# sks-codes/fuzzyheavyhitters

Hardware: AMD Instinct MI355X
Metric: client×prefix key evals/sec (AES blocks/s) + full-crawl wall time, 1M clients (higher is better)
Workload: dtype u32

## Files before the change

fuzzyheavyhitters_amd/csrc/fhh_gc.hip:

```cpp
#include "fhh_internal.h"
#include "aes_keyed.h"
#include "cot_fe.h"
#include "bitslice.h"
#include "gt_window.h"

namespace fhh {

__constant__ WordTable c_T0_gc = T0;
using GcTab = Tab4T32<DevOpsX>;
constexpr int kGcThreads = 1024;

__device__ __forceinline__ void gc_fill(uint32_t* tbl) {
    for (int i = threadIdx.x; i < GcTab::kWords; i += blockDim.x) tbl[i] = GcTab::word(c_T0_gc.v, i);
    __syncthreads();
}

__device__ __forceinline__ void zero_rk(uint32_t (&rk)[11][4]) {
#pragma unroll
    for (int r = 0; r < 11; r++)
#pragma unroll
        for (int c = 0; c < 4; c++) rk[r][c] = ZERO_RK.w[r][c];
}

template <int NB>
// ... 450 lines not shown
                    } else if (t < n_act) {
                        a.gt_msgs[(uint64_t)(r - 1) * n + t] = hl ^ (o ? p1[u] : p0[u]);
                    }
                }
            }
        }
    }
}

template <int B>
__global__ __launch_bounds__(kGcThreads) void k_gt_eval(GcArgs a) {
    __shared__ uint32_t tbl_gc[GcTab::kWords];
    if ((uint64_t)blockIdx.x * kGcThreads >= gc_active(a)) return;
    gc_fill(tbl_gc);
    uint32_t b0, b1;
    GcTab::bases(threadIdx.x & 63, b0, b1);
    const uint64_t n = a.G * a.N;
    const uint64_t Npad = (uint64_t)a.nw * 64;
    const uint64_t n_act = gc_active(a);
    constexpr int U = FHH_GT_EVAL_U;
    const uint64_t stride = (uint64_t)gridDim.x * kGcThreads;
    for (uint64_t t0 = (uint64_t)blockIdx.x * kGcThreads + threadIdx.x; t0 < n_act; t0 += U * stride) {
        uint32_t h[U][4], row[U];
        uint64_t tt[U];
#pragma unroll
        for (int u = 0; u < U; u++) {
            const uint64_t t = t0 + u * stride;
            tt[u] = t;
            const uint64_t tc = t < n_act ? t : t0;
            const uint64_t g = tc / a.N;
            const uint32_t i = (uint32_t)(tc - g * a.N);
            const uint64_t tw = a.gate_base + a.g_off * a.N + tc;
            uint32_t S[4] = {0u, 0u, 0u, 0u}, r = 0;
#pragma unroll
            for (int k = B - 1; k >= 0; k--) {
                uint32_t z[4];
                ld_blk(a.ev_labels, g * B + k, Npad, i, z);
                gf_dbl(S);
#pragma unroll
                for (int c = 0; c < 4; c++) S[c] ^= z[c];
                r |= (z[0] & 1u) << k;
            }
            S[0] ^= (uint32_t)tw;
            S[1] ^= (uint32_t)(tw >> 32);
#pragma unroll
            for (int c = 0; c < 4; c++) h[u][c] = S[c];
            row[u] = r;
        }
        aes0_mmo_tab<DevOpsX, GcTab, U>(h, tbl_gc, b0, b1);
#pragma unroll
        for (int u = 0; u < U; u++) {
            const uint64_t t = tt[u];
            if (t >= n_act) continue;
            const uint64_t hl = (uint64_t)h[u][0] | ((uint64_t)h[u][1] << 32);
            a.sh_ev[t] = row[u] ? (hl ^ a.gt_msgs[(uint64_t)(row[u] - 1) * n + t])
                                : ot_fe_of_u128(hl, (uint64_t)h[u][2] | ((uint64_t)h[u][3] << 32));
        }
    }
}

template <int B>
__global__ __launch_bounds__(kGcThreads) void k_gt_garble_r32(GcArgs a) {
    __shared__ uint32_t tbl_gc[GcTab::kWords];
    if ((uint64_t)blockIdx.x * kGcThreads >= gc_active(a)) return;
    gc_fill(tbl_gc);
    uint32_t b0, b1;
    GcTab::bases(threadIdx.x & 63, b0, b1);
    constexpr uint32_t R = 1u << B;
    constexpr int NB = R < 4 ? (int)R : 4;
    const uint64_t n = a.G * a.N;
    const uint64_t Npad = (uint64_t)a.nw * 64;
    uint32_t* msgs = reinterpret_cast<uint32_t*>(a.gt_msgs);
    uint32_t* vals = reinterpret_cast<uint32_t*>(a.sh_gb);
    uint32_t Dk[B][4];
#pragma unroll
    for (int c = 0; c < 4; c++) Dk[0][c] = a.delta[c];
#pragma unroll
    for (int k = 1; k < B; k++) {
#pragma unroll
        for (int c = 0; c < 4; c++) Dk[k][c] = Dk[k - 1][c];
        gf_dbl(Dk[k]);
    }
    const uint64_t n_act = gc_active(a);
    const uint64_t stride = (uint64_t)gridDim.x * kGcThreads;
    for (uint64_t t = (uint64_t)blockIdx.x * kGcThreads + threadIdx.x; t < n_act; t += stride) {
        const uint64_t g = t / a.N;
        const uint32_t i = (uint32_t)(t - g * a.N);
        const uint64_t tw = a.gate_base + a.g_off * a.N + t;
        uint32_t S[4] = {0u, 0u, 0u, 0u}, col = 0;
#pragma unroll
        for (int k = B - 1; k >= 0; k--) {
            uint32_t z[4];
            ld_blk(a.ev_labels, g * B + k, Npad, i, z);
            const uint32_t xb = plane_bit(a.gb_planes, a.g_off + g, B, k, a.nw, i);
            gf_dbl(S);
#pragma unroll
            for (int c = 0; c < 4; c++) {
                z[c] ^= xb ? 0u : a.delta[c];
                S[c] ^= z[c];
            }
            col |= (z[0] & 1u) << k;
        }
        S[0] ^= (uint32_t)tw;
        S[1] ^= (uint32_t)(tw >> 32);
        const uint32_t rstar = ~col & (R - 1);
        uint32_t p0 = 0, p1 = 0;
#pragma unroll
        for (uint32_t pass = 0; pass < R / NB; pass++) {
            uint32_t h[NB][4];
#pragma unroll
            for (int j = 0; j < NB; j++) {
                const uint32_t flip = (pass * NB + j) ^ col;
#pragma unroll
                for (int c = 0; c < 4; c++) {
                    uint32_t w = S[c];
#pragma unroll
                    for (int k = 0; k < B; k++) w ^= ((flip >> k) & 1u) ? Dk[k][c] : 0u;
                    h[j][c] = w;
                }
            }
            aes0_mmo_tab<DevOpsX, GcTab, NB>(h, tbl_gc, b0, b1);
#pragma unroll
            for (int j = 0; j < NB; j++) {
                const uint32_t r = pass * NB + j;
                const uint32_t o = (uint32_t)(r == rstar) ^ a.mask;
                if (r == 0) {
                    const uint32_t h32 = h[0][0];
                    const uint32_t v = o == 0 ? h32 : (a.mask ? h32 - 1u : h32 + 1u);
                    p0 = v;
                    p1 = a.mask ? v + 1u : v - 1u;
                    vals[t] = a.mask ? v + 1u : v;
                } else {
                    msgs[(uint64_t)(r - 1) * n + t] = h[j][0] ^ (o ? p1 : p0);
                }
            }
        }
    }
}

template <int B>
__global__ __launch_bounds__(kGcThreads) void k_gt_eval_r32(GcArgs a) {
    __shared__ uint32_t tbl_gc[GcTab::kWords];
    if ((uint64_t)blockIdx.x * kGcThreads >= gc_active(a)) return;
    gc_fill(tbl_gc);
    uint32_t b0, b1;
    GcTab::bases(threadIdx.x & 63, b0, b1);
    const uint64_t n = a.G * a.N;
    const uint64_t Npad = (uint64_t)a.nw * 64;
    const uint64_t n_act = gc_active(a);
    const uint32_t* msgs = reinterpret_cast<const uint32_t*>(a.gt_msgs);
    uint32_t* vals = reinterpret_cast<uint32_t*>(a.sh_ev);
    constexpr int U = FHH_GT_EVAL_U;
    const uint64_t stride = (uint64_t)gridDim.x * kGcThreads;
    for (uint64_t t0 = (uint64_t)blockIdx.x * kGcThreads + threadIdx.x; t0 < n_act; t0 += U * stride) {
        uint32_t h[U][4], row[U];
        uint64_t tt[U];
#pragma unroll
        for (int u = 0; u < U; u++) {
            const uint64_t t = t0 + u * stride;
            tt[u] = t;
            const uint64_t tc = t < n_act ? t : t0;
            const uint64_t g = tc / a.N;
            const uint32_t i = (uint32_t)(tc - g * a.N);
            const uint64_t tw = a.gate_base + a.g_off * a.N + tc;
            uint32_t S[4] = {0u, 0u, 0u, 0u}, r = 0;
#pragma unroll
            for (int k = B - 1; k >= 0; k--) {
                uint32_t z[4];
                ld_blk(a.ev_labels, g * B + k, Npad, i, z);
                gf_dbl(S);
#pragma unroll
                for (int c = 0; c < 4; c++) S[c] ^= z[c];
                r |= (z[0] & 1u) << k;
            }
            S[0] ^= (uint32_t)tw;
            S[1] ^= (uint32_t)(tw >> 32);
#pragma unroll
            for (int c = 0; c < 4; c++) h[u][c] = S[c];
            row[u] = r;
        }
        aes0_mmo_tab<DevOpsX, GcTab, U>(h, tbl_gc, b0, b1);
#pragma unroll
        for (int u = 0; u < U; u++) {
            const uint64_t t = tt[u];
            if (t >= n_act) continue;
            vals[t] = row[u] ? (h[u][0] ^ msgs[(uint64_t)(row[u] - 1) * n + t]) : h[u][0];
        }
    }
}

constexpr int kRingSumThreads = 256;
constexpr uint32_t kRingSumSlice = 4096;
__global__ __launch_bounds__(kRingSumThreads) void k_ring32_child_sums(const uint32_t* vals, uint64_t n, uint64_t* sums) {
    const uint64_t c = blockIdx.y;
    const uint64_t lo = (uint64_t)blockIdx.x * kRingSumSlice;
    const uint64_t hi = lo + kRingSumSlice < n ? lo + kRingSumSlice : n;
    const uint32_t* row = vals + c * n;
    uint64_t acc = 0;
    for (uint64_t i = lo + threadIdx.x; i < hi; i += kRingSumThreads) acc += row[i];
#pragma unroll
    for (int off = 32; off > 0; off >>= 1) acc += __shfl_xor(acc, off, 64);
    if ((threadIdx.x & 63) == 0 && acc) atomicAdd(reinterpret_cast<unsigned long long*>(sums + c), (unsigned long long)acc);
}

hipError_t launch_ring32_child_sums(const uint32_t* vals, uint64_t n, uint64_t C, uint64_t* sums, hipStream_t stream) {
    if (n == 0 || C == 0) return hipSuccess;
    if (!vals || !sums) return hipErrorInvalidValue;
    const uint64_t per = (n + kRingSumSlice - 1) / kRingSumSlice;
    for (uint64_t c0 = 0; c0 < C; c0 += 65535) {
        const uint64_t cc = C - c0 < 65535 ? C - c0 : 65535;
        hipLaunchKernelGGL(k_ring32_child_sums, dim3((uint32_t)per, (uint32_t)cc), dim3(kRingSumThreads), 0, stream,
                           vals + c0 * n, n, sums + c0);
        const hipError_t e = hipGetLastError();
        if (e != hipSuccess) return e;
    }
    return hipSuccess;
}

__global__ __launch_bounds__(kRingSumThreads) void k_ring32_child_partials(const uint32_t* vals, uint64_t n, uint64_t c0,
                                                                           const LoopCtl* ctl, uint64_t g_off,
                                                                           uint64_t* partials, uint32_t slot) {
    const uint64_t c = c0 + blockIdx.y;
    if (ctl && (ctl->abort || g_off + c >= ctl->C)) return;
    const uint64_t lo = (uint64_t)blockIdx.x * kRingSumSlice;
    const uint64_t hi = lo + kRingSumSlice < n ? lo + kRingSumSlice : n;
    const uint32_t* row = vals + c * n;
    uint64_t acc = 0;
    for (uint64_t i = lo + threadIdx.x; i < hi; i += kRingSumThreads) acc += row[i];
#pragma unroll
    for (int off = 32; off > 0; off >>= 1) acc += __shfl_xor(acc, off, 64);
    if ((threadIdx.x & 63) == 0 && acc)
        atomicAdd(reinterpret_cast<unsigned long long*>(partials + (g_off + c) * 4 + slot), (unsigned long long)acc);
}

hipError_t launch_ring32_child_partials(const uint32_t* vals, uint64_t n, uint64_t G, const LoopCtl* ctl, uint64_t g_off,
                                        uint64_t* partials, uint32_t slot, hipStream_t stream) {
    if (n == 0 || G == 0) return hipSuccess;
    if (!vals || !partials) return hipErrorInvalidValue;
    const uint64_t per = (n + kRingSumSlice - 1) / kRingSumSlice;
    for (uint64_t c0 = 0; c0 < G; c0 += 65535) {
        const uint64_t cc = G - c0 < 65535 ? G - c0 : 65535;
        hipLaunchKernelGGL(k_ring32_child_partials, dim3((uint32_t)per, (uint32_t)cc), dim3(kRingSumThreads), 0, stream,
                           vals, n, c0, ctl, g_off, partials, slot);
        const hipError_t e = hipGetLastError();
        if (e != hipSuccess) return e;
    }
    return hipSuccess;
}

constexpr int kGtWaves = kGcThreads / 64;

__device__ __forceinline__ void gt_tile_round(uint32_t* st, uint32_t (&x)[32], uint32_t lane, uint32_t (&o)[2][4]) {
#pragma unroll
    for (int kk = 0; kk < 8; kk++) st[64 * kk + (lane ^ (8 * kk))] = x[kk];
    __builtin_amdgcn_wave_barrier();
    const uint32_t kk = lane & 7;
#pragma unroll
    for (int u = 0; u < 2; u++) {
        const uint32_t qq = (lane >> 3) + 8 * u;
        const uint4 v = *reinterpret_cast<const uint4*>(st + 64 * kk + ((4 * qq) ^ (8 * kk)));
        o[u][0] = v.x;
        o[u][1] = v.y;
        o[u][2] = v.z;
        o[u][3] = v.w;
    }
    __builtin_amdgcn_wave_barrier();
#pragma unroll
    for (int i = 0; i < 24; i++) x[i] = x[i + 8];
}

__device__ __forceinline__ void gt_add_partials(uint64_t* partials, uint64_t child, int k0, uint64_t lo, uint64_t hi,
                                                uint32_t lane) {
#pragma unroll
    for (int off = 32; off > 0; off >>= 1) {
        lo += __shfl_xor(lo, off, 64);
        hi += __shfl_xor(hi, off, 64);
    }
    if (lane == 0) {
        atomicAdd(reinterpret_cast<unsigned long long*>(partials + child * 4 + k0), (unsigned long long)lo);
        atomicAdd(reinterpret_cast<unsigned long long*>(partials + child * 4 + k0 + 1), (unsigned long long)hi);
    }
}

__device__ __forceinline__ uint32_t gt_tile_test(uint32_t lane, int r, int u) {
    return 256 * u + 32 * (lane >> 3) + 8 * r + (lane & 7);
}

template <int B>
__device__ __forceinline__ void gt_tile_rows(const GcArgs& a, uint64_t g, uint32_t iw, uint32_t Npt, uint32_t lane,
                                             uint32_t (&x)[32]) {
    static_assert(B >= 1 && B <= kGtTmMaxBits, "gt_tile_rows: b <= 4");
    const uint32_t q = lane >> 2, rg = lane & 3;
    if constexpr (B > kGtTmPadBits) {
        const uint32_t nw2 = 2 * a.nw;
        gt_window_fold<B>(reinterpret_cast<const uint32_t*>(a.ev_labels), g, nw2, gt_window_word(16 * iw + q, nw2), rg, x);
        transpose32(x);
        return;
    }
    const uint32_t* t0 = reinterpret_cast<const uint32_t*>(a.ev_labels) + (((uint64_t)g * B) * Npt + iw) * kGtTileWords + q;
#pragma unroll
    for (int i = 0; i < 32; i++) x[i] = __builtin_nontemporal_load(t0 + (32 * rg + i) * 16);
    if constexpr (B == 2) {
        const uint32_t* t1 = t0 + (uint64_t)Npt * kGtTileWords;
        const uint32_t y0 = __builtin_nontemporal_load(t1 + (rg ? 32 * rg - 1 : 127) * 16);
        x[0] ^= y0;
#pragma unroll
        for (int i = 1; i < 32; i++) x[i] ^= __builtin_nontemporal_load(t1 + (32 * rg + i - 1) * 16);
        if (rg == 0) {
            x[1] ^= y0;
            x[2] ^= y0;
            x[7] ^= y0;
        }
    }
    transpose32(x);
}

template <int B>
__device__ __forceinline__ void gt_tile_colours(const GcArgs& a, uint64_t g, uint32_t iw, uint32_t Npt, uint32_t lane,
                                                uint32_t (&cw)[B][2]) {
    const uint32_t* lab = reinterpret_cast<const uint32_t*>(a.ev_labels);
    if constexpr (B > kGtTmPadBits) {
#pragma unroll
        for (int k = 0; k < B; k++)
#pragma unroll
            for (int u = 0; u < 2; u++) {
                const uint32_t w = gt_window_word(16 * iw + (lane >> 3) + 8 * u, 2 * a.nw);
                cw[k][u] = lab[gt_col_offset(gt_window_col(g, B, k, 2 * a.nw, w))];
            }
        return;
    }
#pragma unroll
    for (int k = 0; k < B; k++)
#pragma unroll
        for (int u = 0; u < 2; u++)
            cw[k][u] = lab[(((uint64_t)g * B + k) * Npt + iw) * kGtTileWords + (lane >> 3) + 8 * u];
}

template <int B>
__device__ __forceinline__ uint32_t gt_row_of(const uint32_t (&cw)[B][2], int r, int u, uint32_t lane) {
    const uint32_t sh = 8 * r + (lane & 7);
    uint32_t row = 0;
#pragma unroll
    for (int k = 0; k < B; k++) row |= ((cw[k][u] >> sh) & 1u) << k;
    return row;
}

template <int B, bool GARBLER>
__device__ __forceinline__ void gt_tile_keys(const GcArgs& a, uint64_t g, uint32_t iw, uint32_t Npt, uint32_t* st,
                                             uint32_t lane, const uint32_t (&Dk)[B][4], uint32_t (&S)[8][4],
                                             uint32_t& col, uint32_t& xcol) {
    if constexpr (B > kGtTmPadBits) {
        xcol = 0;
        col = 0;
        {
            uint32_t ln = lane;
            asm volatile("" : "+v"(ln));
            uint32_t cw[B][2], nx[B][2];
            gt_tile_colours<B>(a, g, iw, Npt, ln, cw);
            if constexpr (GARBLER) {
#pragma unroll
                for (int k = 0; k < B; k++)
#pragma unroll
                    for (int u = 0; u < 2; u++) {
                        const uint32_t w = gt_window_word(16 * iw + (ln >> 3) + 8 * u, 2 * a.nw);
                        nx[k][u] = ~reinterpret_cast<const uint32_t*>(
                            a.gb_planes)[((a.g_off + g) * B + k) * (2 * (uint64_t)a.nw) + w];
                        cw[k][u] ^= nx[k][u];
                    }
            }
#pragma unroll
            for (int r = 0; r < 4; r++)
#pragma unroll
                for (int u = 0; u < 2; u++) {
                    col |= gt_row_of<B>(cw, r, u, ln) << (4 * (2 * r + u));
                    if constexpr (GARBLER) xcol |= gt_row_of<B>(nx, r, u, ln) << (4 * (2 * r + u));
                }
        }
        asm volatile("" : "+v"(col), "+v"(xcol));
        uint32_t x[32];
        gt_tile_rows<B>(a, g, iw, Npt, lane, x);
#pragma unroll 1
        for (int r = 0; r < 4; r++) {
            uint32_t o[2][4];
            gt_tile_round(st, x, lane, o);
#pragma unroll
            for (int j = 0; j < 6; j++)
#pragma unroll
                for (int c = 0; c < 4; c++) S[j][c] = S[j + 2][c];
#pragma unroll
            for (int c = 0; c < 4; c++) {
                S[6][c] = o[0][c];
                S[7][c] = o[1][c];
            }
        }
        return;
    }
    uint32_t x[32], cw[B][2], nx[B][2];
    gt_tile_rows<B>(a, g, iw, Npt, lane, x);
    gt_tile_colours<B>(a, g, iw, Npt, lane, cw);
    if constexpr (GARBLER) {
#pragma unroll
        for (int k = 0; k < B; k++)
#pragma unroll
            for (int u = 0; u < 2; u++) {
                nx[k][u] = ~reinterpret_cast<const uint32_t*>(a.gb_planes)[((a.g_off + g) * B + k) * (2 * (uint64_t)a.nw) +
                                                                          16 * iw + (lane >> 3) + 8 * u];
                cw[k][u] ^= nx[k][u];
            }
    }
    col = 0;
#pragma unroll
    for (int r = 0; r < 4; r++)
#pragma unroll
        for (int u = 0; u < 2; u++) col |= gt_row_of<B>(cw, r, u, lane) << (4 * (2 * r + u));
#pragma unroll 1
    for (int r = 0; r < 4; r++) {
        uint32_t o[2][4];
        gt_tile_round(st, x, lane, o);
        if constexpr (GARBLER) {
#pragma unroll
            for (int u = 0; u < 2; u++)
#pragma unroll
                for (int k = 0; k < B; k++) {
                    const uint32_t f = (nx[k][u] >> (8 * r + (lane & 7))) & 1u;
#pragma unroll
                    for (int c = 0; c < 4; c++) o[u][c] ^= f ? Dk[k][c] : 0u;
                }
        }
#pragma unroll
        for (int j = 0; j < 6; j++)
#pragma unroll
            for (int c = 0; c < 4; c++) S[j][c] = S[j + 2][c];
#pragma unroll
        for (int c = 0; c < 4; c++) {
            S[6][c] = o[0][c];
            S[7][c] = o[1][c];
        }
    }
}

template <int B, bool RING = false>
__global__ __launch_bounds__(kGcThreads) void k_gt_garble_tm(GcArgs a) {
    static_assert(B <= kGtTmMaxBits, "the tile-major garbler takes b <= 4");
    __shared__ uint32_t tbl_gc[GcTab::kWords];
    __shared__ __attribute__((aligned(16))) uint32_t stage[kGtWaves][512];
    const uint32_t lane = threadIdx.x & 63,
                   wv = B > kGtTmPadBits ? (uint32_t)__builtin_amdgcn_readfirstlane((int)(threadIdx.x >> 6)) : threadIdx.x >> 6;
    const uint64_t n_act = gc_active(a);
    const uint32_t Npt = (B > kGtTmPadBits ? a.nw + 7 : a.nw) / 8;
    const uint64_t tiles = (n_act / a.N) * Npt;
    if ((uint64_t)blockIdx.x * kGtWaves >= tiles) return;
    gc_fill(tbl_gc);
    uint32_t b0, b1;
    GcTab::bases(lane, b0, b1);
    constexpr uint32_t R = 1u << B;
    const uint64_t n = a.G * a.N;
    uint32_t Dk[B][4];
#pragma unroll
    for (int c = 0; c < 4; c++) Dk[0][c] = a.delta[c];
#pragma unroll
    for (int k = 1; k < B; k++) {
#pragma unroll
        for (int c = 0; c < 4; c++) Dk[k][c] = Dk[k - 1][c];
        gf_dbl(Dk[k]);
    }
    uint64_t g_next = 0, g_step = 0;
    uint32_t iw_next = 0, iw_step = 0;
    if constexpr (B > kGtTmPadBits) {
        const uint64_t w0 = (uint64_t)blockIdx.x * kGtWaves + wv, ws = (uint64_t)gridDim.x * kGtWaves;
        g_next = w0 / Npt;
        iw_next = (uint32_t)(w0 - g_next * Npt);
        g_step = ws / Npt;
        iw_step = (uint32_t)(ws - g_step * Npt);
    }
    for (uint64_t wt = (uint64_t)blockIdx.x * kGtWaves + wv; wt < tiles; wt += (uint64_t)gridDim.x * kGtWaves) {
        uint64_t g;
        uint32_t iw;
        if constexpr (B > kGtTmPadBits) {
            g = g_next;
            iw = iw_next;
            g_next += g_step;
            iw_next += iw_step;
            if (iw_next >= Npt) {
                iw_next -= Npt;
                g_next++;
            }
        } else {
            g = wt / Npt;
            iw = (uint32_t)(wt - g * Npt);
        }
        uint32_t S[8][4], col, xcol;
        gt_tile_keys<B, true>(a, g, iw, Npt, stage[wv], lane, Dk, S, col, xcol);
        uint64_t acc_lo = 0, acc_hi = 0;
        if constexpr (B > kGtTmPadBits) {
constexpr uint32_t NBW = FHH_GT_TM_WIDE_NB;
#pragma unroll 1
            for (int j = 0; j < 8; j++) {
                const uint32_t i = 512 * iw + gt_tile_test(lane, j >> 1, j & 1);
                const bool live = i < a.N;
                const uint64_t t = g * a.N + i;
                {
                    const uint64_t tw = a.gate_base + a.g_off * a.N + t;
                    S[0][0] ^= (uint32_t)tw;
                    S[0][1] ^= (uint32_t)(tw >> 32);
                }
                const uint32_t cl = col & (R - 1);
                const uint32_t rstar = ~cl & (R - 1);
                typename std::conditional<RING, uint32_t, uint64_t>::type v = 0;
#pragma unroll 1
                for (uint32_t pass = 0; pass < R / NBW; pass++) {
                    uint32_t h[NBW][4];
#pragma unroll
                    for (uint32_t jj = 0; jj < NBW; jj++) {
                        const uint32_t flip = (NBW * pass + jj) ^ cl ^ (xcol & (R - 1));
#pragma unroll
                        for (int c = 0; c < 4; c++) {
                            uint32_t w = S[0][c];
#pragma unroll
                            for (int k = 0; k < B; k++) w ^= ((flip >> k) & 1u) ? Dk[k][c] : 0u;
                            h[jj][c] = w;
                        }
                    }
                    aes0_mmo_tab<DevOpsX, GcTab, NBW>(h, tbl_gc, b0, b1);
#pragma unroll
                    for (uint32_t jj = 0; jj < NBW; jj++) {
                        const uint32_t q = NBW * pass + jj;
                        const uint32_t o_r = (uint32_t)(q == rstar) ^ a.mask;
                        if (jj == 0 && pass == 0) {
                            if constexpr (RING) {
                                const uint32_t h32 = h[0][0];
                                const uint32_t v32 = o_r == 0 ? h32 : (a.mask ? h32 - 1u : h32 + 1u);
                                v = v32;
                                const uint32_t r1 = a.mask ? v32 + 1u : v32;
                                if (live && a.node_partials) acc_lo += r1;
                                else if (live) a.sh_gb[t] = r1;
                            } else {
                                const uint64_t hv = ot_fe_of_u128((uint64_t)h[0][0] | ((uint64_t)h[0][1] << 32),
                                                                  (uint64_t)h[0][2] | ((uint64_t)h[0][3] << 32));
                                v = o_r == 0 ? hv : (a.mask ? fe_dec(hv) : fe_inc(hv));
                                const uint64_t r1 = a.mask ? fe_inc(v) : v;
                                if (live && a.node_partials) {
                                    acc_lo += r1 & 0xFFFFFFFFull;
                                    acc_hi += r1 >> 32;
                                } else if (live) {
                                    a.sh_gb[t] = r1;
                                }
                            }
                        } else if (live) {
                            if constexpr (RING) {
                                const uint32_t v32 = (uint32_t)v;
                                const uint32_t pr = o_r ? (a.mask ? v32 + 1u : v32 - 1u) : v32;
                                reinterpret_cast<uint32_t*>(a.gt_msgs)[(uint64_t)(q - 1) * n + t] = h[jj][0] ^ pr;
                            } else {
                                const uint64_t pr = o_r ? (a.mask ? fe_inc(v) : fe_dec(v)) : v;
                                a.gt_msgs[(uint64_t)(q - 1) * n + t] = ((uint64_t)h[jj][0] | ((uint64_t)h[jj][1] << 32)) ^ pr;
                            }
                        }
                    }
                }
#pragma unroll
                for (int jj = 0; jj < 7; jj++)
#pragma unroll
                    for (int c = 0; c < 4; c++) S[jj][c] = S[jj + 1][c];
                col >>= 4;
                xcol >>= 4;
            }
            if (a.node_partials) gt_add_partials(a.node_partials, a.node_off + a.g_off + g, 0, acc_lo, acc_hi, lane);
            continue;
        }
#pragma unroll 1
        for (int j = 0; j < 8; j++) {
            const uint32_t i = 512 * iw + gt_tile_test(lane, j >> 1, j & 1);
            const bool live = i < a.N;
            const uint64_t t = g * a.N + i;
            const uint64_t tw = a.gate_base + a.g_off * a.N + t;
            const uint32_t K[4] = {S[0][0] ^ (uint32_t)tw, S[0][1] ^ (uint32_t)(tw >> 32), S[0][2], S[0][3]};
            const uint32_t cl = col & (R - 1);
            const uint32_t rstar = ~cl & (R - 1);
            uint32_t h[R][4];
#pragma unroll
            for (uint32_t q = 0; q < R; q++) {
                const uint32_t flip = q ^ cl;
#pragma unroll
                for (int c = 0; c < 4; c++) {
                    uint32_t w = K[c];
#pragma unroll
                    for (int k = 0; k < B; k++) w ^= ((flip >> k) & 1u) ? Dk[k][c] : 0u;
                    h[q][c] = w;
                }
            }
            aes0_mmo_tab<DevOpsX, GcTab, R>(h, tbl_gc, b0, b1);
            uint64_t p0 = 0, p1 = 0;
#pragma unroll
            for (uint32_t q = 0; q < R; q++) {
                const uint32_t o_r = (uint32_t)(q == rstar) ^ a.mask;
                const uint64_t hl = (uint64_t)h[q][0] | ((uint64_t)h[q][1] << 32);
                if (RING && a.ring32) {
                    if (q == 0) {
                        const uint32_t h32 = h[0][0];
                        const uint32_t v = o_r == 0 ? h32 : (a.mask ? h32 - 1u : h32 + 1u);
                        p0 = v;
                        p1 = (uint32_t)(a.mask ? v + 1u : v - 1u);
                        const uint32_t r1 = a.mask ? v + 1u : v;
                        if (live && a.node_partials) acc_lo += r1;
                        else if (live) a.sh_gb[t] = r1;
                    } else if (live) {
                        reinterpret_cast<uint32_t*>(a.gt_msgs)[(uint64_t)(q - 1) * n + t] =
                            h[q][0] ^ (uint32_t)(o_r ? p1 : p0);
                    }
                    continue;
                }
                if (q == 0) {
                    const uint64_t hv = ot_fe_of_u128(hl, (uint64_t)h[q][2] | ((uint64_t)h[q][3] << 32));
                    const uint64_t v = o_r == 0 ? hv : (a.mask ? fe_dec(hv) : fe_inc(hv));
                    p0 = v;
                    p1 = a.mask ? fe_inc(v) : fe_dec(v);
                    const uint64_t r1 = a.mask ? fe_inc(v) : v;
                    if (live && a.node_partials) {
                        acc_lo += r1 & 0xFFFFFFFFull;
                        acc_hi += r1 >> 32;
                    } else if (live) {
                        a.sh_gb[t] = r1;
                    }
                } else if (live) {
                    a.gt_msgs[(uint64_t)(q - 1) * n + t] = hl ^ (o_r ? p1 : p0);
                }
            }
#pragma unroll
            for (int jj = 0; jj < 7; jj++)
#pragma unroll
                for (int c = 0; c < 4; c++) S[jj][c] = S[jj + 1][c];
            col >>= 4;
        }
        if (a.node_partials) gt_add_partials(a.node_partials, a.node_off + a.g_off + g, 0, acc_lo, acc_hi, lane);
    }
}

template <int B>
__global__ __launch_bounds__(kGcThreads) void k_gt_eval_tm(GcArgs a) {
    static_assert(B <= kGtTmMaxBits, "the tile-major evaluator takes b <= 4");
    __shared__ uint32_t tbl_gc[GcTab::kWords];
    __shared__ __attribute__((aligned(16))) uint32_t stage[kGtWaves][512];
    const uint32_t lane = threadIdx.x & 63,
                   wv = B > kGtTmPadBits ? (uint32_t)__builtin_amdgcn_readfirstlane((int)(threadIdx.x >> 6)) : threadIdx.x >> 6;
    const uint64_t n_act = gc_active(a);
    const uint32_t Npt = (B > kGtTmPadBits ? a.nw + 7 : a.nw) / 8;
    const uint64_t tiles = (n_act / a.N) * Npt;
    if ((uint64_t)blockIdx.x * kGtWaves >= tiles) return;
    gc_fill(tbl_gc);
    uint32_t b0, b1;
    GcTab::bases(lane, b0, b1);
    const uint64_t n = a.G * a.N;
    uint64_t g_next = 0, g_step = 0;
    uint32_t iw_next = 0, iw_step = 0;
    if constexpr (B > kGtTmPadBits) {
        const uint64_t w0 = (uint64_t)blockIdx.x * kGtWaves + wv, ws = (uint64_t)gridDim.x * kGtWaves;
        g_next = w0 / Npt;
        iw_next = (uint32_t)(w0 - g_next * Npt);
        g_step = ws / Npt;
        iw_step = (uint32_t)(ws - g_step * Npt);
    }
    for (uint64_t wt = (uint64_t)blockIdx.x * kGtWaves + wv; wt < tiles; wt += (uint64_t)gridDim.x * kGtWaves) {
        uint64_t g;
        uint32_t iw;
        if constexpr (B > kGtTmPadBits) {
            g = g_next;
            iw = iw_next;
            g_next += g_step;
            iw_next += iw_step;
            if (iw_next >= Npt) {
                iw_next -= Npt;
                g_next++;
            }
        } else {
            g = wt / Npt;
            iw = (uint32_t)(wt - g * Npt);
        }
        uint32_t S[8][4], col, xcol;
        const uint32_t nod[B][4] = {};
        gt_tile_keys<B, false>(a, g, iw, Npt, stage[wv], lane, nod, S, col, xcol);
        uint64_t acc_lo = 0, acc_hi = 0;
#pragma unroll 1
        for (int r = 0; r < 4; r++) {
            uint32_t h[2][4];
#pragma unroll
            for (int u = 0; u < 2; u++) {
                const uint32_t i = 512 * iw + gt_tile_test(lane, r, u);
                const uint64_t tw = a.gate_base + a.g_off * a.N + g * a.N + i;
                h[u][0] = S[u][0] ^ (uint32_t)tw;
                h[u][1] = S[u][1] ^ (uint32_t)(tw >> 32);
                h[u][2] = S[u][2];
                h[u][3] = S[u][3];
            }
            aes0_mmo_tab<DevOpsX, GcTab, 2>(h, tbl_gc, b0, b1);
#pragma unroll
            for (int u = 0; u < 2; u++) {
                const uint32_t i = 512 * iw + gt_tile_test(lane, r, u);
                if (i >= a.N) continue;
                const uint64_t t = g * a.N + i;
                const uint32_t row = (col >> (4 * u)) & 0xFu;
                const uint64_t hl = (uint64_t)h[u][0] | ((uint64_t)h[u][1] << 32);
                uint64_t val;
                if (a.ring32)
                    val = row ? (h[u][0] ^ reinterpret_cast<const uint32_t*>(a.gt_msgs)[(uint64_t)(row - 1) * n + t]) : h[u][0];
                else
                    val = row ? (hl ^ a.gt_msgs[(uint64_t)(row - 1) * n + t])
                              : ot_fe_of_u128(hl, (uint64_t)h[u][2] | ((uint64_t)h[u][3] << 32));
                if (a.node_partials) {
                    acc_lo += val & 0xFFFFFFFFull;
                    acc_hi += val >> 32;
                } else {
                    a.sh_ev[t] = val;
                }
            }
#pragma unroll
            for (int jj = 0; jj < 6; jj++)
#pragma unroll
                for (int c = 0; c < 4; c++) S[jj][c] = S[jj + 2][c];
            col >>= 8;
        }
        if (a.node_partials) gt_add_partials(a.node_partials, a.node_off + a.g_off + g, 2, acc_lo, acc_hi, lane);
    }
}

template <int B>
static hipError_t gt_launch(const GcArgs& a, bool garble, hipStream_t stream) {
    int dev = 0, cus = 0;
    hipError_t e = hipGetDevice(&dev);
    if (e != hipSuccess) return e;
    e = hipDeviceGetAttribute(&cus, hipDeviceAttributeMultiprocessorCount, dev);
    if (e != hipSuccess) return e;
    const uint64_t n = a.G * a.N;
    if constexpr (B <= kGtTmMaxBits) if (a.lab_tm) {
        const uint64_t tiles = a.G * ((B > kGtTmPadBits ? a.nw + 7 : a.nw) / 8), need = (tiles + kGtWaves - 1) / kGtWaves;
        const int grid = (int)(need < (uint64_t)cus ? (need ? need : 1) : (uint64_t)cus);
        if (garble && a.ring32) hipLaunchKernelGGL((k_gt_garble_tm<B, true>), dim3(grid), dim3(kGcThreads), 0, stream, a);
        else if (garble) hipLaunchKernelGGL((k_gt_garble_tm<B, false>), dim3(grid), dim3(kGcThreads), 0, stream, a);
        else hipLaunchKernelGGL(k_gt_eval_tm<B>, dim3(grid), dim3(kGcThreads), 0, stream, a);
        return hipGetLastError();
    }
    const uint64_t need = (n + kGcThreads - 1) / kGcThreads;
    const int grid = (int)(need < (uint64_t)cus * 8 ? (need ? need : 1) : (uint64_t)cus * 8);
    if constexpr (B > kGtTmPadBits) if (a.ring32) {
        if (garble) hipLaunchKernelGGL(k_gt_garble_r32<B>, dim3(grid), dim3(kGcThreads), 0, stream, a);
        else hipLaunchKernelGGL(k_gt_eval_r32<B>, dim3(grid), dim3(kGcThreads), 0, stream, a);
        return hipGetLastError();
    }
    if (garble) hipLaunchKernelGGL(k_gt_garble<B>, dim3(grid), dim3(kGcThreads), 0, stream, a);
    else hipLaunchKernelGGL(k_gt_eval<B>, dim3(grid), dim3(kGcThreads), 0, stream, a);
    return hipGetLastError();
}

static hipError_t gt_dispatch(const GcArgs& a, bool garble, hipStream_t stream) {
    if (a.G * a.N == 0) return hipSuccess;
    if (!a.gt_msgs || (!(garble ? a.sh_gb : a.sh_ev) && !(a.lab_tm && a.node_partials)) || !a.ev_labels)
        return hipErrorInvalidValue;
    if (a.lab_tm && (a.bits > (uint32_t)kGtTmMaxBits || (a.bits <= (uint32_t)kGtTmPadBits && a.nw % 8 != 0)))
        return hipErrorInvalidValue;
    if (a.ring32 && !a.lab_tm && a.bits <= (uint32_t)kGtTmPadBits) return hipErrorInvalidValue;
    switch (a.bits) {
        case 1: return gt_launch<1>(a, garble, stream);
        case 2: return gt_launch<2>(a, garble, stream);
        case 3: return gt_launch<3>(a, garble, stream);
        case 4: return gt_launch<4>(a, garble, stream);
        default: return hipErrorInvalidValue;
    }
}

hipError_t launch_gt_garble(const GcArgs& a, hipStream_t stream) { return gt_dispatch(a, true, stream); }

hipError_t launch_gt_eval(const GcArgs& a, hipStream_t stream) { return gt_dispatch(a, false, stream); }

template <int B>
static hipError_t gc_launch(const GcArgs& a, bool garble, hipStream_t stream) {
    int dev = 0, cus = 0;
    hipError_t e = hipGetDevice(&dev);
    if (e != hipSuccess) return e;
    e = hipDeviceGetAttribute(&cus, hipDeviceAttributeMultiprocessorCount, dev);
    if (e != hipSuccess) return e;
    const uint64_t n = a.G * a.N;
    const uint64_t need = (n + kGcThreads - 1) / kGcThreads;
    const int grid = (int)(need < (uint64_t)cus * 8 ? (need ? need : 1) : (uint64_t)cus * 8);
    if (garble && a.ev_ot) hipLaunchKernelGGL(k_gc_garble_cot<B>, dim3(grid), dim3(kGcThreads), 0, stream, a);
    else if (garble) hipLaunchKernelGGL(k_gc_garble<B>, dim3(grid), dim3(kGcThreads), 0, stream, a);
    else if (a.ev_ot) hipLaunchKernelGGL((k_gc_eval<B, true>), dim3(grid), dim3(kGcThreads), 0, stream, a);
    else hipLaunchKernelGGL((k_gc_eval<B, false>), dim3(grid), dim3(kGcThreads), 0, stream, a);
    return hipGetLastError();
}

static hipError_t gc_dispatch(const GcArgs& a, bool garble, hipStream_t stream) {
    if (a.G * a.N == 0) return hipSuccess;
    switch (a.bits) {
        case 1: return gc_launch<1>(a, garble, stream);
        case 2: return gc_launch<2>(a, garble, stream);
        case 3: return gc_launch<3>(a, garble, stream);
        case 4: return gc_launch<4>(a, garble, stream);
        case 5: return gc_launch<5>(a, garble, stream);
        case 6: return gc_launch<6>(a, garble, stream);
        case 7: return gc_launch<7>(a, garble, stream);
        case 8: return gc_launch<8>(a, garble, stream);
        default: return hipErrorInvalidValue;
    }
}

hipError_t launch_gc_garble(const GcArgs& a, hipStream_t stream) { return gc_dispatch(a, true, stream); }

hipError_t launch_gc_eval(const GcArgs& a, hipStream_t stream) { return gc_dispatch(a, false, stream); }

}
```

fuzzyheavyhitters_amd/csrc/fhh_kernels.hip:

```cpp
#include "fhh_internal.h"
#include "expand_kernel.h"
#include "bincode_span.h"
#include "../../include/fhh.h"

namespace fhh {

__constant__ WordTable c_T0 = T0;

__device__ __forceinline__ uint32_t wave_id_uniform() {
    return __builtin_amdgcn_readfirstlane(threadIdx.x >> 6);
}

__device__ __forceinline__ void fill_table(uint32_t* tbl) {
    for (int i = threadIdx.x; i < kTableWords; i += blockDim.x) tbl[i] = c_T0.v[i / kTableReplicas];
    __syncthreads();
}

typedef uint32_t v4u32_t __attribute__((ext_vector_type(4)));
using ExpandTab = Tab4T32<DevOpsX>;
constexpr int kExpandBlock = 1024;

template <bool PAIR, bool NTL>
__device__ __forceinline__ void expand_word(const ExpandJob& J, uint32_t w, uint32_t e_begin, uint32_t e_end,
                                            const uint32_t* tbl, uint32_t lane, uint32_t b0, uint32_t b1) {
    const uint32_t c = w * 64 + lane;
    const size_t npad = J.npad, nw = J.nw;

    const size_t krow = (size_t)J.level * J.K + 2 * J.dim;
    uint4 cw[2];
    uint64_t cwp[2][4];
#pragma unroll
    for (int s = 0; s < 2; s++) {
        cw[s] = J.cw_seed[(krow + s) * npad + c];
#pragma unroll
        for (int b = 0; b < 4; b++) cwp[s][b] = J.cw_bits[((krow + s) * 4 + b) * nw + w];
    }

    for (uint32_t e = e_begin; e < e_end; e++) {
        const uint32_t src = J.live[e];
        uint32_t blk[4][4];
        uint64_t tw[2], yw[2];
        uint64_t pb[4], py[4];
#pragma unroll
        for (int s = 0; s < 2; s++) {
            uint4 sd;
            if constexpr (NTL) {
                const v4u32_t v = __builtin_nontemporal_load(
                    reinterpret_cast<const v4u32_t*>(J.src_seed + ((size_t)src * 2 + s) * npad + c));
                sd = make_uint4(v[0], v[1], v[2], v[3]);
            } else {
                sd = J.src_seed[((size_t)src * 2 + s) * npad + c];
            }
            tw[s] = J.src_t[((size_t)src * 2 + s) * nw + w];
            yw[s] = J.src_y[((size_t)src * 2 + s) * nw + w];
            const uint32_t sw[4] = {sd.x, sd.y, sd.z, sd.w};
#pragma unroll
            for (int dir = 0; dir < 2; dir++) {
                prg_ctr(sw, dir, blk[s * 2 + dir]);
                uint32_t bit, ybit;
                prg_ctrl_bits(blk[s * 2 + dir][0], dir, bit, ybit);
                pb[s * 2 + dir] = __ballot(bit);
                py[s * 2 + dir] = __ballot(ybit);
            }
        }

        if constexpr (PAIR) aes0_mmo_pair<DevOpsX, ExpandTab, 4>(blk, tbl, b0, b1);
        else aes0_mmo_tab<DevOpsX, ExpandTab, 4>(blk, tbl, b0, b1);

#pragma unroll
        for (int s = 0; s < 2; s++) {
            const uint32_t tmask = 0u - (uint32_t)((tw[s] >> lane) & 1);
#pragma unroll
            for (int dir = 0; dir < 2; dir++) {
                const uint32_t* o = blk[s * 2 + dir];
                const v4u32_t out = {o[0] ^ (cw[s].x & tmask), o[1] ^ (cw[s].y & tmask), o[2] ^ (cw[s].z & tmask),
                                     o[3] ^ (cw[s].w & tmask)};
                const size_t de = (size_t)(2 * e + dir) * 2 + s;
                __builtin_nontemporal_store(out, reinterpret_cast<v4u32_t*>(J.dst_seed + de * npad + c));
                if (lane == 0) {
                    J.dst_t[de * nw + w] = pb[s * 2 + dir] ^ (tw[s] & cwp[s][dir]);
                    J.dst_y[de * nw + w] = py[s * 2 + dir] ^ (tw[s] & cwp[s][2 + dir]) ^ yw[s];
                }
            }
        }
    }
}

template <bool PAIR, bool MW, bool NTL>
__global__ __launch_bounds__(kExpandBlock, 1) void k_expand(ExpandLaunch a, uint32_t* work_counter) {
    __shared__ uint32_t tbl[ExpandTab::kWords];
    __shared__ uint32_t s_drained;
    for (int i = threadIdx.x; i < ExpandTab::kWords; i += kExpandBlock) tbl[i] = ExpandTab::word(c_T0.v, i);
    if (threadIdx.x == 0) s_drained = 0;
    __syncthreads();

    const uint32_t lane = threadIdx.x & 63;
    uint32_t b0, b1;
    ExpandTab::bases(lane, b0, b1);
    const uint64_t wpb = kExpandBlock / 64;
    const uint64_t nwaves = (uint64_t)gridDim.x * wpb;
    const LoopCtl* ctl = a.ctl;
    const uint64_t total = ctl ? (ctl->abort ? 0 : ctl->total_items) : a.total_items;
    const uint32_t wpi = MW ? __builtin_amdgcn_readfirstlane(ctl ? ctl->wpi : a.wpi) : 1u;
    constexpr uint32_t H = kExpandHeads;
    uint32_t* heads = work_counter + kExpandSlot0 + (a.seq & 1) * H * kExpandSlotStride;
    if (blockIdx.x == 0 && threadIdx.x < H)
        atomicExch(work_counter + kExpandSlot0 + ((a.seq + 1) & 1) * H * kExpandSlotStride +
                       threadIdx.x * kExpandSlotStride, 0u);
    const uint32_t nh = MW ? (wpi > 1 ? H : 1u) : H;
    const uint32_t home = blockIdx.x & (nh - 1);
    const uint64_t draw_base = MW ? nwaves : 0;
    auto draw = [&]() -> uint64_t {
        uint64_t it = total;
        if (lane == 0) {
            for (uint32_t k = 0; k < nh; k++) {
                const uint32_t h = (home + k) & (nh - 1);
                if ((*(volatile uint32_t*)&s_drained >> h) & 1u) continue;
                const uint32_t v = atomicAdd(heads + h * kExpandSlotStride, 1u);
                const uint64_t cand = draw_base + h + (uint64_t)nh * v;
                if (cand < total) {
                    it = cand;
                    break;
                }
                atomicOr(&s_drained, 1u << h);
            }
        }
        return ((uint64_t)__builtin_amdgcn_readfirstlane((uint32_t)(it >> 32)) << 32) |
               __builtin_amdgcn_readfirstlane((uint32_t)it);
    };
    uint64_t item = MW ? (uint64_t)blockIdx.x * wpb + wave_id_uniform() : draw();
    while (item < total) {
        uint32_t ji = 0;
        if (ctl) {
            while (ji + 1 < a.njobs && item >= ctl->item_begin[ji + 1]) ji++;
        } else {
            while (ji + 1 < a.njobs && item >= a.job[ji + 1].item_begin) ji++;
        }
        ExpandJob J = a.job[ji];
        if (ctl) {
            J.n_live = ctl->n_live[ji % a.jobs_per_ctx];
            J.group = ctl->group;
            J.item_begin = ctl->item_begin[ji];
        }
        const ItemRange r = item_range(item - J.item_begin, J.n_live, J.nw, J.group, wpi);
        for (uint32_t w = r.w0; w < r.w1; w++) expand_word<PAIR, NTL>(J, w, r.e0, r.e1, tbl, lane, b0, b1);
        item = draw();
    }
}

#define FHH_EXPAND_VARIANTS(X)      \
    X(33, false, false, false, 16, 1) \
    X(52, true, true, true, 16, 16)

struct VariantInfo {
    const void* fn;
    int threads;
    uint32_t max_group, max_wpi;
    const char* name;
};

static VariantInfo variant_info(int v) {
    switch (v) {
#define FHH_CASE(id, PAIR, MW, NTL, MAXG, MAXW) \
    case id: return VariantInfo{reinterpret_cast<const void*>(&k_expand<PAIR, MW, NTL>), kExpandBlock, MAXG, MAXW, ExpandTab::kName};
        FHH_EXPAND_VARIANTS(FHH_CASE)
#undef FHH_CASE
        default: return VariantInfo{nullptr, 0, 0, 0, ""};
    }
}

int expand_variant_count() { return 53; }

const char* expand_variant_name(int v) { return variant_info(v).name; }

hipError_t launch_expand(const ExpandLaunch& a0, int variant, int grid, uint32_t* work_counter, uint32_t* seq,
                         hipStream_t stream) {
    if (a0.total_items == 0) return hipSuccess;
    ExpandLaunch a = a0;
    a.seq = *seq;
    const uint64_t wpb = kExpandBlock / 64;
    const uint64_t blocks_needed = (a.total_items + wpb - 1) / wpb;
    const int g = a.ctl ? grid : (int)(blocks_needed < (uint64_t)grid ? blocks_needed : (uint64_t)grid);
    switch (variant) {
#define FHH_CASE(id, PAIR, MW, NTL, MAXG, MAXW) \
    case id: hipLaunchKernelGGL((k_expand<PAIR, MW, NTL>), dim3(g), dim3(kExpandBlock), 0, stream, a, work_counter); break;
        FHH_EXPAND_VARIANTS(FHH_CASE)
#undef FHH_CASE
        default: return hipErrorInvalidValue;
    }
    const hipError_t e = hipGetLastError();
    if (e == hipSuccess) ++*seq;
    return e;
}

int expand_grid(int device, int variant) {
    int cus = 0;
    if (hipDeviceGetAttribute(&cus, hipDeviceAttributeMultiprocessorCount, device) != hipSuccess || cus <= 0) cus = 256;
    const VariantInfo vi = variant_info(variant);
    int per_cu = 0;
    const size_t dyn = 0;
    if (!vi.fn || hipOccupancyMaxActiveBlocksPerMultiprocessor(&per_cu, vi.fn, vi.threads, dyn) != hipSuccess ||
        per_cu <= 0)
        per_cu = 1;
    return cus * per_cu;
}

int expand_threads(int variant) { return variant_info(variant).threads; }
uint32_t expand_max_group(int variant) { return variant_info(variant).max_group; }
uint32_t expand_max_wpi(int variant) { return variant_info(variant).max_wpi; }

__device__ __forceinline__ uint64_t wave_sum_u64(uint64_t v) {
#pragma unroll
    for (int off = 32; off > 0; off >>= 1) v += __shfl_xor(v, off, 64);
    return v;
}

template <int NV>
__device__ __forceinline__ void block_sum_u64(uint64_t (&v)[NV], uint64_t* red ) {
    const int lane = threadIdx.x & 63, wid = threadIdx.x >> 6, nwv = blockDim.x >> 6;
#pragma unroll
    for (int k = 0; k < NV; k++) v[k] = wave_sum_u64(v[k]);
    if (lane == 0)
#pragma unroll
        for (int k = 0; k < NV; k++) red[k * (kReduceThreads / 64) + wid] = v[k];
    __syncthreads();
    if (threadIdx.x == 0) {
#pragma unroll
        for (int k = 0; k < NV; k++) {
            uint64_t s = 0;
            for (int i = 0; i < nwv; i++) s += red[k * (kReduceThreads / 64) + i];
            v[k] = s;
        }
    }
    __syncthreads();
}

__device__ __forceinline__ uint64_t child_count(const ChildArgs& a) {
    return a.ctl ? (a.ctl->abort ? 0 : a.ctl->C) : a.C;
}

__device__ __forceinline__ uint64_t child_end(const ChildArgs& a) {
    const uint64_t C = child_count(a);
    if (!a.c_cnt) return C;
    const uint64_t e = a.c_off + a.c_cnt;
    return e < C ? e : C;
}

__device__ __forceinline__ void child_entries(const ChildArgs& a, uint64_t c, uint32_t (&e)[kMaxDims]) {
    const uint64_t p = c >> a.d;
    const uint32_t i = (uint32_t)(c & ((1u << a.d) - 1));
#pragma unroll
    for (int j = 0; j < kMaxDims; j++)
        if (j < (int)a.d) e[j] = 2 * a.parent_pos[p * a.d + j] + ((i >> j) & 1);
}

__device__ __forceinline__ uint64_t eq_word(const ChildArgs& a, const uint32_t (&e)[kMaxDims], uint32_t w) {
    uint64_t m = a.valid[w];
#pragma unroll
    for (int j = 0; j < kMaxDims; j++) {
        if (j < (int)a.d) {
#pragma unroll
            for (int s = 0; s < 2; s++) {
                const size_t idx = ((size_t)e[j] * 2 + s) * a.nw + w;
                const uint64_t e0 = a.s0.t[j][idx] ^ a.s0.y[j][idx];
                const uint64_t e1 = a.s1.t[j][idx] ^ a.s1.y[j][idx];
                m &= ~(e0 ^ e1);
            }
        }
    }
    return m;
}

constexpr int kEqThreads = 1024;
__global__ __launch_bounds__(kEqThreads) void k_eq_count(ChildArgs a, uint64_t* counts) {
    __shared__ uint64_t red[kEqThreads / 64];
    const uint64_t C_ = child_count(a);
    for (uint64_t c = blockIdx.x; c < C_; c += gridDim.x) {
        uint32_t e[kMaxDims];
        child_entries(a, c, e);
        uint64_t v[1] = {0};
        for (uint32_t w = threadIdx.x; w < a.nw; w += 2 * kEqThreads) {
            const uint32_t w1 = w + kEqThreads;
            const uint64_t m0 = eq_word(a, e, w);
            const uint64_t m1 = w1 < a.nw ? eq_word(a, e, w1) : 0;
            v[0] += __popcll(m0) + __popcll(m1);
        }
        block_sum_u64<1>(v, red);
        if (threadIdx.x == 0) counts[c] = v[0];
    }
}

static int child_grid(uint64_t C) { return (int)(C < 65535 ? (C ? C : 1) : 65535); }
static uint64_t window_cap(const ChildArgs& a) { return a.c_cnt && a.c_cnt < a.C ? a.c_cnt : a.C; }

hipError_t launch_eq_count(const ChildArgs& a, uint64_t* counts, hipStream_t stream) {
    if (a.C == 0) return hipSuccess;
    hipLaunchKernelGGL(k_eq_count, dim3(child_grid(a.C)), dim3(kEqThreads), 0, stream, a, counts);
    return hipGetLastError();
}

__global__ __launch_bounds__(kReduceThreads) void k_share_planes(ChildArgs a, uint64_t* out) {
    const uint64_t C_ = child_end(a);
    for (uint64_t c = a.c_off + blockIdx.x; c < C_; c += gridDim.x) {
        uint32_t e[kMaxDims];
        child_entries(a, c, e);
        const uint32_t pnw = a.plane_nw ? a.plane_nw : a.nw;
        for (uint32_t w = threadIdx.x; w < pnw; w += blockDim.x) {
#pragma unroll
            for (int s = 0; s < 2; s++)
#pragma unroll
                for (int j = 0; j < kMaxDims; j++)
                    if (j < (int)a.d) {
                        const size_t idx = ((size_t)e[j] * 2 + s) * a.nw + w;
                        out[((size_t)(c - a.c_off) * 2 * a.d + (size_t)s * a.d + j) * pnw + w] =
                            w < a.nw ? (a.s0.t[j][idx] ^ a.s0.y[j][idx]) & a.valid[w] : 0ull;
                    }
        }
    }
}

hipError_t launch_share_planes(const ChildArgs& a, uint64_t* out, hipStream_t stream) {
    if (a.C == 0) return hipSuccess;
    hipLaunchKernelGGL(k_share_planes, dim3(child_grid(window_cap(a))), dim3(kReduceThreads), 0, stream, a, out);
    return hipGetLastError();
}

__device__ __forceinline__ uint64_t mix64(uint64_t z) {
    z += 0x9e3779b97f4a7c15ull;
    z = (z ^ (z >> 30)) * 0xbf58476d1ce4e5b9ull;
    z = (z ^ (z >> 27)) * 0x94d049bb133111ebull;
    return z ^ (z >> 31);
}

constexpr uint64_t kFeP = (1ull << 62) - (1ull << 30) - 1;

__device__ __forceinline__ bool sim_eq_bit(const ChildArgs& a, const uint32_t (&e)[kMaxDims], uint64_t c, uint32_t i) {
    if (a.gc_out) return ((a.gc_out[(c - a.c_off) * a.gc_N + i] ^ a.gc_mask) & 1u) != 0;
    return (eq_word(a, e, i >> 6) >> (i & 63)) & 1;
}

constexpr uint32_t kSimOtChunk = 16 * kReduceThreads;
__global__ __launch_bounds__(kReduceThreads) void k_child_sums_fe(ChildArgs a, uint64_t* partials) {
    __shared__ uint64_t red[4 * (kReduceThreads / 64)];
    const uint64_t base = mix64(a.prf_seed ^ a.level);
    const uint64_t C_ = child_end(a);
    const uint32_t i_begin = blockIdx.y * kSimOtChunk;
    const uint32_t i_end = min(i_begin + kSimOtChunk, a.n);
    for (uint64_t c = a.c_off + blockIdx.x; c < C_; c += gridDim.x) {
        uint32_t e[kMaxDims];
        child_entries(a, c, e);
        const uint64_t bc = mix64(base ^ c);
        uint64_t v[4] = {0, 0, 0, 0};
        for (uint32_t i = i_begin + threadIdx.x; i < i_end; i += blockDim.x) {
            uint64_t r1, v1;
            if (a.ot_val[0]) {
                const size_t t = (c - a.c_off) * a.gc_N + i;
                r1 = static_cast<const uint64_t*>(a.ot_val[0])[t];
                v1 = static_cast<const uint64_t*>(a.ot_val[1])[t];
            } else {
                uint64_t r0 = mix64(mix64(bc ^ (a.client_base + i)) ^ 0ull) & ((1ull << 62) - 1);
                if (r0 >= kFeP) r0 -= kFeP;
                r1 = (r0 + 1 == kFeP) ? 0 : r0 + 1;
                v1 = sim_eq_bit(a, e, c, i) ? r0 : r1;
            }
            v[0] += r1 & 0xFFFFFFFFull;
            v[1] += r1 >> 32;
            v[2] += v1 & 0xFFFFFFFFull;
            v[3] += v1 >> 32;
        }
        block_sum_u64<4>(v, red);
        if (threadIdx.x == 0)
            for (int k = 0; k < 4; k++) atomicAdd(reinterpret_cast<unsigned long long*>(partials + c * 4 + k), v[k]);
    }
}

hipError_t launch_child_sums_fe(const ChildArgs& a, uint64_t* partials, hipStream_t stream, bool zero) {
    if (a.C == 0) return hipSuccess;
    if (zero) {
        const hipError_t e = hipMemsetAsync(partials, 0, (size_t)a.C * 4 * sizeof(uint64_t), stream);
        if (e != hipSuccess) return e;
    }
    const uint32_t chunks = a.n ? (a.n + kSimOtChunk - 1) / kSimOtChunk : 1;
    hipLaunchKernelGGL(k_child_sums_fe, dim3(child_grid(window_cap(a)), chunks), dim3(kReduceThreads), 0, stream, a,
                       partials);
    return hipGetLastError();
}

// ... 691 lines not shown
```

Before: 103.0 billion.

## Prefetch next-iteration loads in expand and GT eval; use scalar loads for uniform data

The expand kernel now loads the next live entry's seeds and control words while the current AES batch runs, and reads wave-uniform arrays (live, t/y bits, cw_bits) through the constant address space so they become scalar loads. The GT evaluator preloads all eight OT message words for a tile before the first AES round instead of loading inside each round. The B==2 tile-row load now issues all loads before the XOR behind a scheduling barrier, and wv uses readfirstlane unconditionally. These hide global-memory latency behind AES work at the cost of more live registers, which may lower occupancy.

```diff
diff --git a/fuzzyheavyhitters_amd/csrc/fhh_gc.hip b/fuzzyheavyhitters_amd/csrc/fhh_gc.hip
--- a/fuzzyheavyhitters_amd/csrc/fhh_gc.hip
+++ b/fuzzyheavyhitters_amd/csrc/fhh_gc.hip
@@ -776,10 +776,14 @@
     for (int i = 0; i < 32; i++) x[i] = __builtin_nontemporal_load(t0 + (32 * rg + i) * 16);
     if constexpr (B == 2) {
         const uint32_t* t1 = t0 + (uint64_t)Npt * kGtTileWords;
-        const uint32_t y0 = __builtin_nontemporal_load(t1 + (rg ? 32 * rg - 1 : 127) * 16);
-        x[0] ^= y0;
-#pragma unroll
-        for (int i = 1; i < 32; i++) x[i] ^= __builtin_nontemporal_load(t1 + (32 * rg + i - 1) * 16);
+        uint32_t y[32];
+        y[0] = __builtin_nontemporal_load(t1 + (rg ? 32 * rg - 1 : 127) * 16);
+#pragma unroll
+        for (int i = 1; i < 32; i++) y[i] = __builtin_nontemporal_load(t1 + (32 * rg + i - 1) * 16);
+        __builtin_amdgcn_sched_barrier(0);
+        const uint32_t y0 = y[0];
+#pragma unroll
+        for (int i = 0; i < 32; i++) x[i] ^= y[i];
         if (rg == 0) {
             x[1] ^= y0;
             x[2] ^= y0;
@@ -918,8 +922,7 @@
     static_assert(B <= kGtTmMaxBits, "the tile-major garbler takes b <= 4");
     __shared__ uint32_t tbl_gc[GcTab::kWords];
     __shared__ __attribute__((aligned(16))) uint32_t stage[kGtWaves][512];
-    const uint32_t lane = threadIdx.x & 63,
-                   wv = B > kGtTmPadBits ? (uint32_t)__builtin_amdgcn_readfirstlane((int)(threadIdx.x >> 6)) : threadIdx.x >> 6;
+    const uint32_t lane = threadIdx.x & 63, wv = (uint32_t)__builtin_amdgcn_readfirstlane((int)(threadIdx.x >> 6));
     const uint64_t n_act = gc_active(a);
     const uint32_t Npt = (B > kGtTmPadBits ? a.nw + 7 : a.nw) / 8;
     const uint64_t tiles = (n_act / a.N) * Npt;
@@ -1115,8 +1118,7 @@
     static_assert(B <= kGtTmMaxBits, "the tile-major evaluator takes b <= 4");
     __shared__ uint32_t tbl_gc[GcTab::kWords];
     __shared__ __attribute__((aligned(16))) uint32_t stage[kGtWaves][512];
-    const uint32_t lane = threadIdx.x & 63,
-                   wv = B > kGtTmPadBits ? (uint32_t)__builtin_amdgcn_readfirstlane((int)(threadIdx.x >> 6)) : threadIdx.x >> 6;
+    const uint32_t lane = threadIdx.x & 63, wv = (uint32_t)__builtin_amdgcn_readfirstlane((int)(threadIdx.x >> 6));
     const uint64_t n_act = gc_active(a);
     const uint32_t Npt = (B > kGtTmPadBits ? a.nw + 7 : a.nw) / 8;
     const uint64_t tiles = (n_act / a.N) * Npt;
@@ -1154,8 +1156,29 @@
         const uint32_t nod[B][4] = {};
         gt_tile_keys<B, false>(a, g, iw, Npt, stage[wv], lane, nod, S, col, xcol);
         uint64_t acc_lo = 0, acc_hi = 0;
-#pragma unroll 1
-        for (int r = 0; r < 4; r++) {
+        constexpr bool EARLY = B <= kGtTmPadBits;
+        uint64_t m[8] = {};
+        if constexpr (EARLY) {
+            uint64_t at[8];
+#pragma unroll
+            for (int j = 0; j < 8; j++) {
+                const uint32_t i = 512 * iw + gt_tile_test(lane, j >> 1, j & 1);
+                const uint32_t row = (col >> (4 * j)) & 0xFu;
+                at[j] = row != 0 && i < a.N ? (uint64_t)(row - 1) * n + g * a.N + i : 0;
+            }
+            if (a.ring32) {
+#pragma unroll
+                for (int j = 0; j < 8; j++) {
+                    uint32_t z = 0;
+                    asm volatile("" : "+v"(z));
+                    m[j] = reinterpret_cast<const uint32_t*>(a.gt_msgs)[at[j]] | ((uint64_t)z << 32);
+                }
+            } else {
+#pragma unroll
+                for (int j = 0; j < 8; j++) m[j] = a.gt_msgs[at[j]];
+            }
+        }
+        auto round = [&](int r) __attribute__((always_inline)) {
             uint32_t h[2][4];
 #pragma unroll
             for (int u = 0; u < 2; u++) {
@@ -1167,6 +1190,14 @@
                 h[u][3] = S[u][3];
             }
             aes0_mmo_tab<DevOpsX, GcTab, 2>(h, tbl_gc, b0, b1);
+            const uint64_t mr[2] = {m[0], m[1]};
+            if constexpr (EARLY) {
+#pragma unroll
+                for (int jj = 0; jj < 6; jj++) {
+                    m[jj] = m[jj + 2];
+                    asm volatile("" : "+v"(m[jj]) : "v"(h[0][0]));
+                }
+            }
 #pragma unroll
             for (int u = 0; u < 2; u++) {
                 const uint32_t i = 512 * iw + gt_tile_test(lane, r, u);
@@ -1176,9 +1207,11 @@
                 const uint64_t hl = (uint64_t)h[u][0] | ((uint64_t)h[u][1] << 32);
                 uint64_t val;
                 if (a.ring32)
-                    val = row ? (h[u][0] ^ reinterpret_cast<const uint32_t*>(a.gt_msgs)[(uint64_t)(row - 1) * n + t]) : h[u][0];
+                    val = row ? (h[u][0] ^ (EARLY ? (uint32_t)mr[u]
+                                                  : reinterpret_cast<const uint32_t*>(a.gt_msgs)[(uint64_t)(row - 1) * n + t]))
+                              : h[u][0];
                 else
-                    val = row ? (hl ^ a.gt_msgs[(uint64_t)(row - 1) * n + t])
+                    val = row ? (hl ^ (EARLY ? mr[u] : a.gt_msgs[(uint64_t)(row - 1) * n + t]))
                               : ot_fe_of_u128(hl, (uint64_t)h[u][2] | ((uint64_t)h[u][3] << 32));
                 if (a.node_partials) {
                     acc_lo += val & 0xFFFFFFFFull;
@@ -1192,7 +1225,10 @@
 #pragma unroll
                 for (int c = 0; c < 4; c++) S[jj][c] = S[jj + 2][c];
             col >>= 8;
-        }
+        };
+        if constexpr (EARLY) round(0);
+#pragma unroll 1
+        for (int r = EARLY ? 1 : 0; r < 4; r++) round(r);
         if (a.node_partials) gt_add_partials(a.node_partials, a.node_off + a.g_off + g, 2, acc_lo, acc_hi, lane);
     }
 }
diff --git a/fuzzyheavyhitters_amd/csrc/fhh_kernels.hip b/fuzzyheavyhitters_amd/csrc/fhh_kernels.hip
--- a/fuzzyheavyhitters_amd/csrc/fhh_kernels.hip
+++ b/fuzzyheavyhitters_amd/csrc/fhh_kernels.hip
@@ -20,11 +20,29 @@
 using ExpandTab = Tab4T32<DevOpsX>;
 constexpr int kExpandBlock = 1024;
 
+#ifndef FHH_EXPAND_SLOAD
+#define FHH_EXPAND_SLOAD 1
+#endif
+#ifndef FHH_EXPAND_PREFETCH
+#define FHH_EXPAND_PREFETCH 1
+#endif
+
+template <typename T>
+__device__ __forceinline__ T uniform_load(const T* p, size_t i) {
+#if FHH_EXPAND_SLOAD
+    return ((const __attribute__((address_space(4))) T*)p)[i];
+#else
+    return p[i];
+#endif
+}
+
 template <bool PAIR, bool NTL>
 __device__ __forceinline__ void expand_word(const ExpandJob& J, uint32_t w, uint32_t e_begin, uint32_t e_end,
                                             const uint32_t* tbl, uint32_t lane, uint32_t b0, uint32_t b1) {
+    constexpr bool kPrefetch = FHH_EXPAND_PREFETCH, kAhead = FHH_EXPAND_SLOAD || FHH_EXPAND_PREFETCH;
     const uint32_t c = w * 64 + lane;
     const size_t npad = J.npad, nw = J.nw;
+    if (e_begin >= e_end) return;
 
     const size_t krow = (size_t)J.level * J.K + 2 * J.dim;
     uint4 cw[2];
@@ -33,27 +51,41 @@
     for (int s = 0; s < 2; s++) {
         cw[s] = J.cw_seed[(krow + s) * npad + c];
 #pragma unroll
-        for (int b = 0; b < 4; b++) cwp[s][b] = J.cw_bits[((krow + s) * 4 + b) * nw + w];
-    }
-
-    for (uint32_t e = e_begin; e < e_end; e++) {
-        const uint32_t src = J.live[e];
-        uint32_t blk[4][4];
-        uint64_t tw[2], yw[2];
-        uint64_t pb[4], py[4];
+        for (int b = 0; b < 4; b++) cwp[s][b] = uniform_load(J.cw_bits, ((krow + s) * 4 + b) * nw + w);
+    }
+
+    uint4 sd[2];
+    uint64_t tw[2], yw[2];
+    auto fetch = [&](uint32_t src) __attribute__((always_inline)) {
 #pragma unroll
         for (int s = 0; s < 2; s++) {
-            uint4 sd;
             if constexpr (NTL) {
                 const v4u32_t v = __builtin_nontemporal_load(
                     reinterpret_cast<const v4u32_t*>(J.src_seed + ((size_t)src * 2 + s) * npad + c));
-                sd = make_uint4(v[0], v[1], v[2], v[3]);
+                sd[s] = make_uint4(v[0], v[1], v[2], v[3]);
             } else {
-                sd = J.src_seed[((size_t)src * 2 + s) * npad + c];
-            }
-            tw[s] = J.src_t[((size_t)src * 2 + s) * nw + w];
-            yw[s] = J.src_y[((size_t)src * 2 + s) * nw + w];
-            const uint32_t sw[4] = {sd.x, sd.y, sd.z, sd.w};
+                sd[s] = J.src_seed[((size_t)src * 2 + s) * npad + c];
+            }
+            tw[s] = uniform_load(J.src_t, ((size_t)src * 2 + s) * nw + w);
+            yw[s] = uniform_load(J.src_y, ((size_t)src * 2 + s) * nw + w);
+        }
+    };
+    uint32_t src = kAhead ? uniform_load(J.live, e_begin) : 0u;
+    if constexpr (kPrefetch) {
+        fetch(src);
+        asm volatile("" ::"v"(cw[0].x), "v"(cw[1].x));
+    }
+
+    for (uint32_t e = e_begin; e < e_end; e++) {
+        if constexpr (!kAhead) src = J.live[e];
+        if constexpr (!kPrefetch) fetch(src);
+        const bool more = e + 1 < e_end;
+        if (kAhead && more) src = uniform_load(J.live, e + 1);
+        uint32_t blk[4][4];
+        uint64_t pb[4], py[4];
+#pragma unroll
+        for (int s = 0; s < 2; s++) {
+            const uint32_t sw[4] = {sd[s].x, sd[s].y, sd[s].z, sd[s].w};
 #pragma unroll
             for (int dir = 0; dir < 2; dir++) {
                 prg_ctr(sw, dir, blk[s * 2 + dir]);
@@ -67,22 +99,31 @@
         if constexpr (PAIR) aes0_mmo_pair<DevOpsX, ExpandTab, 4>(blk, tbl, b0, b1);
         else aes0_mmo_tab<DevOpsX, ExpandTab, 4>(blk, tbl, b0, b1);
 
+        v4u32_t out[4];
+        uint64_t tq[4], yq[4];
 #pragma unroll
         for (int s = 0; s < 2; s++) {
             const uint32_t tmask = 0u - (uint32_t)((tw[s] >> lane) & 1);
 #pragma unroll
             for (int dir = 0; dir < 2; dir++) {
                 const uint32_t* o = blk[s * 2 + dir];
-                const v4u32_t out = {o[0] ^ (cw[s].x & tmask), o[1] ^ (cw[s].y & tmask), o[2] ^ (cw[s].z & tmask),
-                                     o[3] ^ (cw[s].w & tmask)};
-                const size_t de = (size_t)(2 * e + dir) * 2 + s;
-                __builtin_nontemporal_store(out, reinterpret_cast<v4u32_t*>(J.dst_seed + de * npad + c));
-                if (lane == 0) {
-                    J.dst_t[de * nw + w] = pb[s * 2 + dir] ^ (tw[s] & cwp[s][dir]);
-                    J.dst_y[de * nw + w] = py[s * 2 + dir] ^ (tw[s] & cwp[s][2 + dir]) ^ yw[s];
-                }
-            }
-        }
+                out[2 * dir + s] = v4u32_t{o[0] ^ (cw[s].x & tmask), o[1] ^ (cw[s].y & tmask), o[2] ^ (cw[s].z & tmask),
+                                           o[3] ^ (cw[s].w & tmask)};
+                tq[2 * dir + s] = pb[s * 2 + dir] ^ (tw[s] & cwp[s][dir]);
+                yq[2 * dir + s] = py[s * 2 + dir] ^ (tw[s] & cwp[s][2 + dir]) ^ yw[s];
+            }
+        }
+        if (lane == 0) {
+#pragma unroll
+            for (int q = 0; q < 4; q++) {
+                J.dst_t[((size_t)4 * e + q) * nw + w] = tq[q];
+                J.dst_y[((size_t)4 * e + q) * nw + w] = yq[q];
+            }
+        }
+        if (kPrefetch && more) fetch(src);
+#pragma unroll
+        for (int q = 0; q < 4; q++)
+            __builtin_nontemporal_store(out[q], reinterpret_cast<v4u32_t*>(J.dst_seed + ((size_t)4 * e + q) * npad + c));
     }
 }
 
```

Result: faster. 104.4 billion (median of 6 runs) (+1.4%).
